# AllenNeuralDynamics/aind-smartspim-destripe

Measured on AMD Instinct MI355X. Metric: 2048x2048 uint16 slices/s destriped, higher is better.
Workload: dtype f32

## Files before the change

### aind_smartspim_destripe_amd/csrc/dsx.hip

```cpp
#include <hip/hip_runtime.h>
#include <dlfcn.h>
#include <math.h>
#include <rccl/rccl.h>
#include <stdio.h>
#include <stdlib.h>
#include <string.h>

#include <string>
#include <vector>

#include "../../include/dsx.h"
#include "dsx_kernels.h"
#include "dsx_retile.h"
#include "dsx_pyramid.h"
#include "dsx_wavelet.h"
#include "dsx_plan.h"
#include "dsx_io.h"
#include "dsx_streaks.h"
#include "dsx_zenc_kernels.h"
#include "dsx_lz4enc_kernels.h"
#include "dsx_zdec_kernels.h"

namespace {

thread_local std::string g_init_error;

enum KernelClass { KC_FWD1 = 0, KC_FWD, KC_HIST, KC_OTSU, KC_ROW, KC_INV, KC_FINAL, KC_COUNT };
const char* kClassNames[KC_COUNT] = {"k_fwd_march(level1)", "k_fwd_march(coarse)", "k_hist", "k_otsu",
                                     "k_rowfilter",       "k_inv_march(pyramid)", "k_inv_march(final)"};

struct ProfRec {
  int cls;
  hipEvent_t e0, e1;
};

}

struct DsxTuning {
  int row_wpb = 0;
  int march_waves = 256 * 16;
  bool no_quant = false;
  int seg_min_rows = 4;
  bool no_fuse = false;
  bool no_fuse_inv = false;
  bool no_pair = false;
  int hist_rows = 0;
  int fwd_wpb = 8, inv_wpb = 8;
  bool no_row_multi = false;
  int row_multi_alone = 48;
  int helper = -1;
  bool no_pipeline = false;
#ifdef DSX_DIAG
  int skip_hist = 0, skip_row = 0, skip_from = 1000;
#endif
};

struct dsx_ctx {
  int device = 0;
  DsxTuning tune;
  hipStream_t stream_ = nullptr;
  std::string err;
  bool planned = false;
  dsx::Plan plan;
  dsx::HostCfg cfg[2];
  double high_int = 2700.0;
  int max_batch = 0;
// ... 27 lines not shown
  int wl_bank_len = 0;
  bool wl_set = false;
  float wl[4][dsx::kMaxTaps] = {};
  float wl_bank[4][dsx::kMaxTaps] = {};
  unsigned* h_sticky = nullptr;
  uint8_t* zenc_slots = nullptr;
  uint32_t* zenc_sizes = nullptr;
  size_t zenc_blocks = 0;
  uint8_t* zenc_lits = nullptr;
  size_t zenc_lit_blocks = 0;
  uint8_t* zdec_scratch = nullptr;
  size_t zdec_bytes = 0;
  unsigned* d_sticky = nullptr;
  bool stack_mode = false;
  bool no_fuse_rf = false;
  bool fuse_rf_wide = false;
  int ablate = 0;
  static constexpr int kMaxStreams = 8;
  int n_streams = 4;
  hipStream_t aux[kMaxStreams] = {};
  hipEvent_t ev_fork = nullptr, ev_join[kMaxStreams] = {};
  hipStream_t helper[kMaxStreams] = {};
  hipEvent_t ev_h[kMaxStreams][4] = {};
  int joins_pending = 0;
  unsigned long long main_ops = 0;
  struct {
    const void* in = nullptr; void* out = nullptr; const void* cfg = nullptr;
    int n = 0, in_dtype = 0, out_dtype = 0, parts = 0;
    unsigned long long main_ops = 0;
  } last_split;
// ... 64 lines not shown
  t.row_wpb = env_int("DSX_ROW_WPB", 0);
  if (t.row_wpb != 0) t.row_wpb = std::max(4, std::min(t.row_wpb, (int)dsx::kRowMaxWaves));
  t.march_waves = std::max(64, env_int("DSX_MARCH_WAVES", 256 * 16));
  t.no_quant = env_int("DSX_NO_QUANT", 0) != 0;
  t.seg_min_rows = std::max(2, env_int("DSX_SEG_MIN_ROWS", 4));
  t.no_fuse = env_int("DSX_NO_FUSE", 0) != 0;
  t.no_fuse_inv = env_int("DSX_NO_FUSE_INV", 0) != 0;
  t.no_pair = env_int("DSX_NO_PAIR", 0) != 0;
  t.hist_rows = std::max(0, env_int("DSX_HIST_ROWS", 0));
  t.fwd_wpb = env_int("DSX_FWD_WPB", 8) == 4 ? 4 : 8;
  t.inv_wpb = env_int("DSX_INV_WPB", 8) == 4 ? 4 : 8;
  t.no_row_multi = env_int("DSX_NO_ROW_MULTI", 0) != 0;
  t.row_multi_alone = std::max(0, env_int("DSX_ROW_MULTI_ALONE", 48));
  t.helper = getenv("DSX_HELPER") ? (env_int("DSX_HELPER", 0) != 0 ? 1 : 0) : -1;
  t.no_pipeline = env_int("DSX_NO_PIPELINE", 0) != 0;
#ifdef DSX_DIAG
  t.skip_hist = env_int("DSX_SKIP_HIST", 0);
  t.skip_row = env_int("DSX_SKIP_ROW", 0);
  t.skip_from = env_int("DSX_SKIP_COARSE", 1000);
#endif
}

int fail(dsx_ctx* c, int code, const std::string& msg) {
  if (c) c->err = msg;
  else g_init_error = msg;
  return code;
}

hipStream_t use_main(dsx_ctx* c) {
  for (int i = 1; i < c->joins_pending; ++i) (void)hipStreamWaitEvent(c->stream_, c->ev_join[i], 0);
// ... 52 lines not shown
    }
  }
};

int rowfilter_waves_per_block(int M) {
  int best_w = 4, best_total = 0;
  for (int w = 4; w <= dsx::kRowMaxWaves; ++w) {
    const size_t bytes = (size_t)M * (w + 1) * sizeof(float2);
    const int blocks = (int)std::min<size_t>(160 * 1024 / bytes, 8);
    const int total = std::min(blocks * w, 16);
    if (total > best_total) { best_total = total; best_w = w; }
  }
  return best_w;
}

template <int CPL, int GF = -1, int NT = -1, int HALO = -1, int PLAN = 0>
hipError_t launch_rowfilter(const dsx::RowArgs& a_in, int npairs, int nb, hipStream_t s) {
  static bool attr_set[64] = {};
  int dev = 0;
  (void)hipGetDevice(&dev);
  if (!attr_set[dev & 63]) {
    hipError_t e = hipFuncSetAttribute((const void*)dsx::k_rowfilter<CPL, GF, NT, HALO, PLAN>,
                                       hipFuncAttributeMaxDynamicSharedMemorySize, 160 * 1024);
    if (e != hipSuccess) return e;
    attr_set[dev & 63] = true;
  }
  int force_wpb = tune().row_wpb;
  if (force_wpb && (size_t)a_in.M * (force_wpb + 1) * sizeof(float2) > 160 * 1024) force_wpb = 0;
  const int wpb = force_wpb ? force_wpb : ((CPL > 18 || a_in.M >= 1024) ? 4 : rowfilter_waves_per_block(a_in.M));
  const size_t smem = (size_t)a_in.M * (wpb + 1) * sizeof(float2);
  const dsx::RowArgs& a = a_in;
  const dim3 grid((npairs + wpb - 1) / wpb, nb);
  hipLaunchKernelGGL((dsx::k_rowfilter<CPL, GF, NT, HALO, PLAN>), grid, dim3(64 * wpb), smem, s, a);
  return hipGetLastError();
}

hipError_t launch_rowfilter_wide(const dsx::RowArgs& a, int npairs, int nb, hipStream_t s) {
  static bool attr_set[64] = {};
  int dev = 0;
  (void)hipGetDevice(&dev);
  if (!attr_set[dev & 63]) {
    hipError_t e = hipFuncSetAttribute((const void*)dsx::k_rowfilter_wide, hipFuncAttributeMaxDynamicSharedMemorySize,
                                       (int)(dsx::kWideMaxLen * sizeof(float2)));
    if (e != hipSuccess) return e;
    attr_set[dev & 63] = true;
  }
  if (a.M > dsx::kWideMaxLen || a.w >= 65536) return hipErrorInvalidValue;
  hipLaunchKernelGGL(dsx::k_rowfilter_wide, dim3(npairs, nb), dim3(dsx::kWideThreads), (size_t)a.M * sizeof(float2), s, a);
  return hipGetLastError();
}

hipError_t dispatch_rowfilter(const dsx::RowArgs& a, int npairs, int nb, hipStream_t s) {
  const int cpl = (a.M + 63) / 64;
  if (cpl > 36) return launch_rowfilter_wide(a, npairs, nb, s);
  const int gf = a.w >> 8, nt = (a.w - (gf << 8) + 63) >> 6;
  auto plan_is = [&](int m, int r0, int r1, int r2) {
    return a.M == m && a.npass == 3 && a.radix[0] == r0 && a.radix[1] == r1 && a.radix[2] == r2;
  };
  if (cpl <= 2) return launch_rowfilter<2>(a, npairs, nb, s);
  if (cpl <= 4) return launch_rowfilter<4>(a, npairs, nb, s);
  if (cpl <= 6) return launch_rowfilter<6>(a, npairs, nb, s);
  if (cpl <= 10) return launch_rowfilter<10>(a, npairs, nb, s);
  if (cpl <= 18) {
    if (gf == 4 && nt == 1 && a.K == 0) {
      if (plan_is(1026, 19, 9, 6))
        return launch_rowfilter<18, 4, 1, 0, 1>(a, npairs, nb, s);
      return launch_rowfilter<18, 4, 1, 0>(a, npairs, nb, s);
    }
    if (gf == 2 && nt == 1 && a.K > 0) {
      if (plan_is(1071, 17, 9, 7))
        return launch_rowfilter<18, 2, 1, 1, 2>(a, npairs, nb, s);
      return launch_rowfilter<18, 2, 1, 1>(a, npairs, nb, s);
    }
    if (gf == 1 && nt == 4 && a.K > 0) {
      if (plan_is(1024, 16, 8, 8)) return launch_rowfilter<18, 1, 4, 1, 5>(a, npairs, nb, s);
      if (plan_is(960, 15, 8, 8)) return launch_rowfilter<18, 1, 4, 1, 6>(a, npairs, nb, s);
    }
    return launch_rowfilter<18>(a, npairs, nb, s);
  }
  if (a.K > 0 && gf == 3) {
    if (nt == 4 && plan_is(2048, 16, 16, 8)) return launch_rowfilter<36, 3, 4, 1, 3>(a, npairs, nb, s);
    if (nt == 3 && plan_is(1815, 15, 11, 11)) return launch_rowfilter<36, 3, 3, 1, 4>(a, npairs, nb, s);
  }
  return launch_rowfilter<36>(a, npairs, nb, s);
}

int rowfinal_plan(const dsx::Plan& p, const dsx::LevelPlan& lp, int in_dtype, int out_dtype, bool pair_io, bool wide) {
  if (!pair_io || in_dtype != DSX_U16 || out_dtype != DSX_U16) return 0;
  if ((lp.w & 1) != 0 || (p.Wout + dsx::kMarchCols - 1) / dsx::kMarchCols > dsx::kRfWaves) return 0;
  const int gf = lp.w >> 8, nt = (lp.w - (gf << 8) + 63) >> 6;
  auto plan_is = [&](int m, int r0, int r1, int r2) {
    return lp.M == m && lp.npass == 3 && lp.radix[0] == r0 && lp.radix[1] == r1 && lp.radix[2] == r2;
  };
  if (gf == 4 && nt == 1 && lp.K == 0 && plan_is(1026, 19, 9, 6)) return 1;
  if (wide && lp.K > 0 && gf == 3 && nt == 4 && plan_is(2048, 16, 16, 8)) return 3;
  if (wide && lp.K > 0 && gf == 3 && nt == 3 && plan_is(1815, 15, 11, 11)) return 4;
  return 0;
}

template <int CPL, int GF, int NT, int HALO, int PLAN>
hipError_t launch_rowfinal_t(const dsx::RowFinalArgs& a, int nb, hipStream_t s) {
  static bool attr_set[64] = {};
  int dev = 0;
  (void)hipGetDevice(&dev);
  auto kern = dsx::k_rowfinal<CPL, GF, NT, HALO, PLAN>;
  if (!attr_set[dev & 63]) {
    hipError_t e = hipFuncSetAttribute((const void*)kern, hipFuncAttributeMaxDynamicSharedMemorySize, 160 * 1024);
    if (e != hipSuccess) return e;
    attr_set[dev & 63] = true;
  }
  const size_t smem = (size_t)a.r.M * (dsx::kRfWaves + 1) * sizeof(float2);
  const int np = (a.f.hout + 1) / 2;
  int nblk = (np + dsx::kRfRows - 1) / dsx::kRfRows;
#if DSX_RF_XCD
  nblk = (nblk + 7) / 8 * 8;
#endif
  const dim3 grid(nblk, nb);
  hipLaunchKernelGGL(kern, grid, dim3(64 * dsx::kRfWaves), smem, s, a);
  return hipGetLastError();
}

hipError_t launch_rowfinal(int plan, const dsx::RowFinalArgs& a, int nb, hipStream_t s) {
  if (plan == 1) return launch_rowfinal_t<18, 4, 1, 0, 1>(a, nb, s);
  if (plan == 3) return launch_rowfinal_t<36, 3, 4, 1, 3>(a, nb, s);
  if (plan == 4) return launch_rowfinal_t<36, 3, 3, 1, 4>(a, nb, s);
  return hipErrorInvalidValue;
}

hipError_t launch_rowfilter_multi(const dsx::RowMultiArgs& a_in, const int* npairs, int nb, hipStream_t s) {
  static bool attr_set[64] = {};
  int dev = 0;
  (void)hipGetDevice(&dev);
  if (!attr_set[dev & 63]) {
    hipError_t e = hipFuncSetAttribute((const void*)dsx::k_rowfilter_multi<6>, hipFuncAttributeMaxDynamicSharedMemorySize, 160 * 1024);
    if (e != hipSuccess) return e;
    attr_set[dev & 63] = true;
  }
  const int wpb = dsx::kRowMaxWaves;
  dsx::RowMultiArgs a = a_in;
  int blocks = 0, max_m = 1;
// ... 264 lines not shown
    a.kcut[1] = lp.kcut[1];
    a.inv_M = 1.0f / (float)lp.M;
    a.ablate = ctx->ablate;
    if (fuse_rf && l == 0) {
      row1 = a;
      continue;
    }
    const int npairs = (lp.h + 1) / 2;
    const int multi_alone = ctx->tune.row_multi_alone;
    if (!no_multi && (!v.alone || nb <= multi_alone) && rs == s && a.M <= 6 * 64 && multi.nlev < dsx::kRowMultiMax) {
      multi_pairs[multi.nlev] = npairs;
      multi.lv[multi.nlev++] = a;
      continue;
    }
    LaunchScope ls(ctx, KC_ROW);
    DSX_HIP(dispatch_rowfilter(a, npairs, nb, rs));
  }
  if (multi.nlev == 1) {
    LaunchScope ls(ctx, KC_ROW);
    DSX_HIP(dispatch_rowfilter(multi.lv[0], multi_pairs[0], nb, s));
  } else if (multi.nlev > 1) {
    LaunchScope ls(ctx, KC_ROW);
    DSX_HIP(launch_rowfilter_multi(multi, multi_pairs, nb, s));
  }
  if (split_inv) DSX_HIP(hipEventRecord(v.ev[3], v.helper));
  if (ctx->stop_after == 2) return DSX_OK;

  for (int l = L - 1; l >= (L > 0 ? 0 : -1); --l) {
    if (fuse21 && l == 1) continue;
    if (l >= skip_from) continue;
    if (generic) {
// ... 77 lines not shown
      f.has_c2 = (L > 2) ? 1 : 0;
      f.has_c = 1;
      f.pair_io = pair_io ? 1 : 0;
      if (f.rows_per_seg & 1) {
        f.rows_per_seg += 1;
        f.nseg = ((f.hout + 1) / 2 + f.rows_per_seg - 1) / f.rows_per_seg;
      }
    }
    dim3 grid((f.nstrips * f.nseg + 3) / 4, nb);
    LaunchScope ls(ctx, last ? KC_FINAL : KC_INV);
    const int inv_wpb = ctx->tune.inv_wpb;
    if (fused && fuse_rf) {
      dsx::RowFinalArgs rf;
      rf.r = row1;
      rf.f = f;
      DSX_HIP(launch_rowfinal(rf_plan, rf, nb, s));
    } else if (fused && inv_wpb == 8) {
      const dim3 g8((f.nstrips * f.nseg + 7) / 8, nb);
      if (in_dtype == DSX_U16) hipLaunchKernelGGL((dsx::k_inv_march<0, true, 8>), g8, dim3(512), 0, s, f);
      else hipLaunchKernelGGL((dsx::k_inv_march<1, true, 8>), g8, dim3(512), 0, s, f);
    } else if (fused) {
      if (in_dtype == DSX_U16) hipLaunchKernelGGL((dsx::k_inv_march<0, true>), grid, dim3(256), 0, s, f);
      else hipLaunchKernelGGL((dsx::k_inv_march<1, true>), grid, dim3(256), 0, s, f);
    } else if (!last) {
      hipLaunchKernelGGL(dsx::k_inv_march<2>, grid, dim3(256), 0, s, f);
    } else if (in_dtype == DSX_U16) {
      hipLaunchKernelGGL(dsx::k_inv_march<0>, grid, dim3(256), 0, s, f);
    } else {
      hipLaunchKernelGGL(dsx::k_inv_march<1>, grid, dim3(256), 0, s, f);
    }
    DSX_HIP(hipGetLastError());
// ... 336 lines not shown
  return DSX_OK;
}

}

extern "C" {

int dsx_device_count(void) {
  int n = 0;
  if (hipGetDeviceCount(&n) != hipSuccess) return 0;
  return n;
}

const char* dsx_last_error(const dsx_ctx* ctx) { return ctx ? ctx->err.c_str() : g_init_error.c_str(); }

int dsx_init(int device, dsx_ctx** out_ctx) {
  if (!out_ctx) { g_init_error = "out_ctx is NULL"; return DSX_EINVAL; }
  *out_ctx = nullptr;
  int n = 0;
  hipError_t e = hipGetDeviceCount(&n);
  if (e != hipSuccess || n <= 0) {
    g_init_error = std::string("no HIP device available: ") + hipGetErrorString(e);
    return DSX_EHIP;
  }
  if (device < 0 || device >= n) { g_init_error = "device index out of range"; return DSX_EINVAL; }
  e = hipSetDevice(device);
  if (e != hipSuccess) { g_init_error = std::string("hipSetDevice: ") + hipGetErrorString(e); return DSX_EHIP; }
  dsx_ctx* c = new dsx_ctx();
  c->device = device;
  read_tuning(c->tune);
// ... 117 lines not shown
  if (bank) {
    memcpy(ctx->wl, ctx->wl_bank, sizeof(ctx->wl));
    const void* fns[6] = {(const void*)dsx::k_fwd_gen<0>, (const void*)dsx::k_fwd_gen<1>, (const void*)dsx::k_fwd_gen<2>,
                          (const void*)dsx::k_inv_gen<0>, (const void*)dsx::k_inv_gen<1>, (const void*)dsx::k_inv_gen<2>};
    for (const void* fn : fns)
      DSX_HIP(hipFuncSetAttribute(fn, hipFuncAttributeMaxDynamicSharedMemorySize, 160 * 1024));
  }
  const std::string perr = dsx::build_plan(height, width, ctx->cfg, ctx->plan, bank ? ctx->wl_bank_len : dsx::kFilterLen);
  if (!perr.empty()) {
    const bool limit = perr.find("too") != std::string::npos;
    return fail(ctx, limit ? DSX_ELIMIT : DSX_EINVAL, perr);
  }
  const dsx::Plan& p = ctx->plan;
  ctx->high_int = microscope_high_int;
  ctx->max_batch = max_batch;
  const int L = p.L, Lc = L > 0 ? L : 1;

  const size_t ws_bytes = (size_t)max_batch * p.plane_floats * sizeof(float);
  DSX_HIP(hipMalloc((void**)&ctx->d_ws, ws_bytes));
  const size_t stats_b = sizeof(dsx::PlaneStats) * max_batch;
  const size_t minmax_b = sizeof(unsigned) * 2 * Lc * max_batch;
  const size_t hist_b = sizeof(unsigned) * 256 * Lc * max_batch;
  ctx->ctl_zero_bytes = stats_b + minmax_b + hist_b;
  DSX_HIP(hipMalloc((void**)&ctx->d_ctl, ctx->ctl_zero_bytes));
  ctx->d_stats = (dsx::PlaneStats*)ctx->d_ctl;
  ctx->d_minmax = (unsigned*)(ctx->d_ctl + stats_b);
  ctx->d_hist = (unsigned*)(ctx->d_ctl + stats_b + minmax_b);
  DSX_HIP(hipMalloc((void**)&ctx->d_thr, sizeof(float) * Lc * max_batch));
  DSX_HIP(hipMalloc((void**)&ctx->d_otsu, sizeof(float) * Lc * max_batch));
  DSX_HIP(hipMalloc((void**)&ctx->d_cfg, sizeof(int) * max_batch));
// ... 1116 lines not shown
```

### aind_smartspim_destripe_amd/csrc/dsx_kernels.h

```cpp
#ifndef DSX_KERNELS_H
#define DSX_KERNELS_H

#include <type_traits>
#include <hip/hip_runtime.h>
#include <stdint.h>

#include "dsx_fft_core.h"

#ifndef DSX_NT
#define DSX_NT 1
#endif
#ifndef DSX_MEDIAN_BALLOT
#define DSX_MEDIAN_BALLOT 1
#endif
#ifndef DSX_FWD_STEADY
#define DSX_FWD_STEADY 1
#endif
#ifndef DSX_RF_XCD
#define DSX_RF_XCD 0
#endif
#ifndef DSX_INV_MINW
#define DSX_INV_MINW 1
#endif
#ifndef DSX_FWD_PRUNE
// ... 1356 lines not shown
    if ((c >> 16) <= rank_b) rb = tb;
  }
  return ra | (rb << 16);
}

template <int CPL>
constexpr int row_waves_per_simd() {
  return CPL <= 18 ? 4 : 1;
}
constexpr int kRowMaxWaves = 8;

__host__ __device__ __forceinline__ constexpr int rf_lds_row_b(int M) { return (M + 1) & ~1; }

template <int CPL, int GF_, int NT_, int HALO_, int PLAN_, bool TO_LDS>
__device__ __forceinline__ void rf_pair_body(const RowArgs& a, float2* s_tw, float2* buf, int tid, int nthreads, int lane,
                                             int pair, int plane) {
  const int M = (PLAN_ > 0) ? StaticFft<PLAN_>::M : a.M;
  constexpr bool SWZ = StaticFft<PLAN_>::kSwz;
  auto P = [](int i) { return SWZ ? dsx_idx_swz::at(i) : i; };
  const int N = a.w, K = (HALO_ == 0) ? 0 : a.K;
  const bool halo = (HALO_ >= 0) ? (HALO_ != 0) : (K > 0);
  const int npairs = (a.h + 1) >> 1;
  const bool live = pair < npairs;
  const int r0 = live ? 2 * pair : 0;
  const bool has_b = (r0 + 1) < a.h;
  const int cfg = a.cfg[plane];
  float* rowa = a.ws + plane * a.ws_plane_stride + a.da_off + (long long)r0 * a.ld;
  float* rowb = rowa + a.ld;

  constexpr int GV = RowSlots<CPL>::GV;
  constexpr int E = RowSlots<CPL>::E;
// ... 27 lines not shown
    rb4[g] = make_float4(0.f, 0.f, 0.f, 0.f);
    if (active && g < gf) {
      ra4[g] = *(const float4*)(rowa + 256 * g + 4 * lane);
      if (has_b) rb4[g] = *(const float4*)(rowb + 256 * g + 4 * lane);
    }
  }
#pragma unroll
  for (int k = 0; k < 4; ++k) {
    rta[k] = 0.f;
    rtb[k] = 0.f;
    if (active && k < nt && tn + 64 * k < N) {
      rta[k] = rowa[tn + 64 * k];
      if (has_b) rtb[k] = rowb[tn + 64 * k];
    }
  }
  for (int i = tid; i < M; i += nthreads) s_tw[P(i)] = a.tw[i];
  __syncthreads();
  float* const lds_a = (float*)buf;
  float* const lds_b = (float*)buf + rf_lds_row_b(M);
  if (!active) {
    if (TO_LDS) {
      for (int n = 2 * lane; n < N; n += 2 * kWave) {
        *(float2*)(lds_a + n) = make_float2(0.f, 0.f);
        *(float2*)(lds_b + n) = make_float2(0.f, 0.f);
      }
    }
    return;
  }

  float va[E], vb[E];
  mask_t maska = 0, maskb = 0;
  auto take = [&](int e, float xa, float xb, bool valid) {
// ... 225 lines not shown
#endif
    }
  }
#pragma unroll
  for (int k = 0; k < 4; ++k) {
    const int n = tn + 64 * k;
    if (k < nt && n < N) {
      const int e = 4 * GV + k;
      const float2 y = buf[P(K + n)];
      rowa[n] = bit_select(slot_mask(maska, e), 0.f, -y.y * a.inv_M);
      if (has_b) rowb[n] = bit_select(slot_mask(maskb, e), 0.f, -y.x * a.inv_M);
    }
  }
}

template <int CPL, int GF_ = -1, int NT_ = -1, int HALO_ = -1, int PLAN_ = 0>
__global__ __launch_bounds__(64 * kRowMaxWaves, row_waves_per_simd<CPL>()) void k_rowfilter(RowArgs a) {
  extern __shared__ __attribute__((aligned(16))) float2 dsx_smem[];
  const int tid = threadIdx.x, lane = tid & 63, wave = tid >> 6;
  const int M = (PLAN_ > 0) ? StaticFft<PLAN_>::M : a.M;
  rf_pair_body<CPL, GF_, NT_, HALO_, PLAN_, false>(a, dsx_smem, dsx_smem + (long long)M * (1 + wave), tid, blockDim.x, lane,
                                                   blockIdx.x * (blockDim.x >> 6) + wave, blockIdx.y);
}

constexpr int kRowMultiMax = 8;
struct RowMultiArgs {
  int nlev;
  int blk_end[kRowMultiMax];
  RowArgs lv[kRowMultiMax];
};

template <int CPL>
__global__ __launch_bounds__(64 * kRowMaxWaves, row_waves_per_simd<CPL>()) void k_rowfilter_multi(RowMultiArgs args) {
  extern __shared__ __attribute__((aligned(16))) float2 dsx_smem[];
  const int tid = threadIdx.x, lane = tid & 63, wave = tid >> 6;
  int ent = 0;
  while (ent + 1 < args.nlev && (int)blockIdx.x >= args.blk_end[ent]) ++ent;
  const RowArgs& a = args.lv[ent];
  const int bx = (int)blockIdx.x - (ent > 0 ? args.blk_end[ent - 1] : 0);
  rf_pair_body<CPL, -1, -1, -1, 0, false>(a, dsx_smem, dsx_smem + (long long)a.M * (1 + wave), tid, blockDim.x, lane,
                                          bx * (blockDim.x >> 6) + wave, blockIdx.y);
}

constexpr int kWideThreads = 512;
constexpr int kWideCpl = 36;
constexpr int kWideMaxLen = kWideThreads * kWideCpl;

__device__ __forceinline__ unsigned wide_block_sum(unsigned v, unsigned* s_red, int& turn) {
  v = __reduce_add_sync(~0ull, v);
  unsigned* slot = s_red + ((turn & 1) ? (kWideThreads / 64) : 0);
  if ((threadIdx.x & 63) == 0) slot[threadIdx.x >> 6] = v;
  __syncthreads();
  unsigned t = 0;
#pragma unroll
  for (int w = 0; w < kWideThreads / 64; ++w) t += slot[w];
  ++turn;
// ... 669 lines not shown
  if (IN_KIND != 2 && a.flat != nullptr) {
    if (fast) inv_march_body<IN_KIND, true, IN_KIND != 2>(a, lane, strip, seg, plane);
    else inv_march_body<IN_KIND, false, IN_KIND != 2>(a, lane, strip, seg, plane);
  } else {
    if (fast) inv_march_body<IN_KIND, true, false>(a, lane, strip, seg, plane);
    else inv_march_body<IN_KIND, false, false>(a, lane, strip, seg, plane);
  }
}

constexpr int kRfWaves = 8;
constexpr int kRfRows = 2 * kRfWaves - 2;

struct RowFinalArgs {
  RowArgs r;
  FinalArgs f;
};

struct RowFinalPre {
  uint4 ni[2];

};

template <bool SHADE, bool PREFETCH_ONLY = false>
__device__ __forceinline__ void rowfinal_synth(const FinalArgs& a, const float2* smem, int M, int lane, int strip, int plane,
                                               int p_begin, int p_end, int row0, RowFinalPre& pre) {
  constexpr float RL0[6] = DSX_REC_LO;
  constexpr float RH0[6] = DSX_REC_HI;
  constexpr float KS = 1.44269504088896340736f;
  constexpr float RL[6] = {RL0[0] * KS, RL0[1] * KS, RL0[2] * KS, RL0[3] * KS, RL0[4] * KS, RL0[5] * KS};
  constexpr float RH[6] = {RH0[0] * KS, RH0[1] * KS, RH0[2] * KS, RH0[3] * KS, RH0[4] * KS, RH0[5] * KS};
// ... 152 lines not shown
    if (gyl < a.hout && x0 < a.wout)
      __builtin_amdgcn_raw_buffer_store_b128(o4, rs_out, vo_pair_out, (unsigned)(2 * p * a.wout) * 2u, kBufNT);
  };
  for (int p = p_begin; p < p_end; p += 3) {
    const bool more = p + 3 < p_end;
    step(p, ni[0], A[0], A[1], A[2], D[0], D[1], D[2]);
    if (more) ni[0] = issue_i(2 * (p + 3));
    if (p + 1 < p_end) step(p + 1, ni[1], A[1], A[2], A[0], D[1], D[2], D[0]);
    if (more) ni[1] = issue_i(2 * (p + 4));
    if (p + 2 < p_end) step(p + 2, ni[2], A[2], A[0], A[1], D[2], D[0], D[1]);
    if (more) ni[2] = issue_i(2 * (p + 5));
  }
}

template <int CPL, int GF_, int NT_, int HALO_, int PLAN_>
__global__ __launch_bounds__(64 * kRfWaves, CPL <= 18 ? 4 : 2) void k_rowfinal(RowFinalArgs a) {
  extern __shared__ __attribute__((aligned(16))) float2 dsx_smem[];
  const int tid = threadIdx.x, lane = tid & 63;
  const int wave = __builtin_amdgcn_readfirstlane(tid >> 6);
  constexpr int M = StaticFft<PLAN_>::M;
  const int plane = blockIdx.y;
#if DSX_RF_XCD
  const int per_die = gridDim.x >> 3;
  const int bx = (blockIdx.x & 7) * per_die + (blockIdx.x >> 3);
#else
  const int bx = blockIdx.x;
#endif
  const int pair0 = (kRfWaves - 1) * bx;
  rf_pair_body<CPL, GF_, NT_, HALO_, PLAN_, true>(a.r, dsx_smem, dsx_smem + (long long)M * (1 + wave), tid, 64 * kRfWaves, lane,
                                                  pair0 + wave, plane);
  const int np = (a.f.hout + 1) >> 1;
  const int p_begin = 2 * pair0, p_end = min(np, p_begin + kRfRows);
  const bool synth = wave < a.f.nstrips && p_begin < p_end;
  RowFinalPre pre;
  asm volatile("" ::: "memory");
  __builtin_amdgcn_sched_barrier(0);
  if (synth) rowfinal_synth<false, true>(a.f, dsx_smem, M, lane, wave, plane, p_begin, p_end, 2 * pair0, pre);
  __syncthreads();
  if (!synth) return;
  if (a.f.flat != nullptr) rowfinal_synth<true>(a.f, dsx_smem, M, lane, wave, plane, p_begin, p_end, 2 * pair0, pre);
  else rowfinal_synth<false>(a.f, dsx_smem, M, lane, wave, plane, p_begin, p_end, 2 * pair0, pre);
}

}
#endif
```

### aind_smartspim_destripe_amd/csrc/dsx_plan.h

```cpp
#ifndef DSX_PLAN_H
#define DSX_PLAN_H

#include <math.h>
#include <stdint.h>
#include <stdlib.h>

#include <algorithm>
#include <string>
#include <vector>

namespace dsx {

constexpr int kPlanMaxLevels = 16;
constexpr int kPlanMaxPasses = 16;
constexpr int kFilterLen = 6;
constexpr int kMaxFftLen = 64 * 36;
constexpr int kMaxWideLen = 512 * 36;

struct HostCfg {
  int level;
  double sigma;
  double max_threshold;
};

// ... 249 lines not shown
      int kc = 0;
      for (int k = 0; k < M; ++k) {
        const double mag = std::max(fabs((double)g1[k].re), sqrt((double)g2[k].re * g2[k].re + (double)g2[k].im * g2[k].im));
        if (mag > 1e-9) kc = std::max(kc, std::min(k, M - k));
      }
      lp.kcut[c] = kc;
      p.consts.insert(p.consts.end(), g1.begin(), g1.end());
      p.consts.insert(p.consts.end(), g2.begin(), g2.end());
    }
  }
  p.plane_floats = (off + 3) & ~3LL;
  if (p.plane_floats == 0) p.plane_floats = 4;
  return "";
}

}
#endif
```

### aind_smartspim_destripe_amd/engine.py

```python

import ctypes
import math
import os

import numpy as np

from . import wavelets

_HERE = os.path.dirname(os.path.abspath(__file__))
LIB_PATH = os.environ.get("DSX_LIB") or os.path.join(_HERE, "_lib", "libdsx_hip.so")

DSX_U16, DSX_F32 = 0, 1
DSX_WAVELET_DB3 = 3
DSX_WAVELET_BANK = 0
STAGE_APPROX, STAGE_DETAIL = 0, 1
STREAM_COMPUTE, STREAM_UPLOAD, STREAM_DOWNLOAD = 0, 1, 2

TASK_FILL, TASK_COPY, TASK_STORED, TASK_ZSTD, TASK_LZ4 = 0, 1, 2, 3, 4
TASK_ZLIB, TASK_BLOSCLZ = 5, 6
TASK_SHUFFLE, TASK_SPLIT, TASK_BITSHUFFLE = 0x100, 0x200, 0x400
ZDEC_ZSTD, ZDEC_ANY, ZDEC_ALL = 0, 1, 3
ROUTE_DEVICE, ROUTE_HOST, ROUTE_FILL = 0, 1, 2
TASK_DTYPE = np.dtype([("src", "<u8"), ("dst", "<u8"), ("src_len", "<u4"), ("dst_len", "<u4"), ("kind", "<u4"),
                       ("chunk", "<u4")])
# ... 7 lines not shown
    "dsx_set_shading_device", "dsx_constants_device", "dsx_run_host", "dsx_run_device", "dsx_sync",
    "dsx_malloc", "dsx_free", "dsx_memcpy_h2d", "dsx_memcpy_d2h", "dsx_memcpy_d2d",
    "dsx_timer_start", "dsx_timer_stop", "dsx_profile_enable", "dsx_profile_read",
    "dsx_get_stats", "dsx_get_thresholds", "dsx_get_level", "dsx_set_stop_after", "dsx_set_stack_mode",
    "dsx_bricks_to_planes_u16", "dsx_planes_to_bricks_u16", "dsx_downsample2_u16",
    "dsx_flatfield_correction", "dsx_flatfield_correction_rows", "dsx_foreground_background",
    "dsx_comm_unique_id", "dsx_comm_init", "dsx_comm_destroy", "dsx_comm_broadcast", "dsx_comm_allreduce_f64",
    "dsx_malloc_host", "dsx_free_host", "dsx_memcpy_h2d_async", "dsx_memcpy_d2h_async",
    "dsx_stream_wait", "dsx_stream_sync", "dsx_event_record", "dsx_event_sync",
    "dsx_io_read_chunks", "dsx_io_write_chunks", "dsx_io_write_chunks_blosc", "dsx_blosc_decode", "dsx_blosc_encode",
    "dsx_png_unfilter", "dsx_plan_streaks", "dsx_plan_streaks_ex", "dsx_get_streaks_threshold",
    "dsx_blosc_encode_device", "dsx_blosc_encode_ref", "dsx_blosc_encode_device_ex", "dsx_blosc_encode_ref_ex",
    "dsx_io_read_frames", "dsx_io_read_frames_ex", "dsx_blosc_decode_device", "dsx_blosc_decode_ref",
    "dsx_io_read_zlib_chunks", "dsx_io_write_chunks_blosc_lz4", "dsx_blosc_encode_lz4",
    "dsx_pyramid_work_bytes", "dsx_pyramid_block_u16", "dsx_pyramid_block_ref",
    "dsx_pyramid_bricks_u16", "dsx_pyramid_bricks_ref",
]


def frame_tasks_per_chunk(chunk_bytes):
    return int(chunk_bytes) // 8192 + 1


def decode_task(src, dst, src_len, dst_len, kind, chunk=0):
    t = np.zeros(1, TASK_DTYPE)
    t[0] = (src, dst, src_len, dst_len, kind, chunk)
    return t


class DsxError(RuntimeError):

# ... 134 lines not shown
    lib.dsx_blosc_encode_ref_ex.argtypes = [vp, i32, ctypes.c_size_t, i32, i32, vp, vp, i32]
    lib.dsx_io_read_frames.argtypes = [vp, ctypes.POINTER(ctypes.c_char_p), i32, ctypes.c_size_t, i32, ctypes.c_uint16,
                                       vp, ctypes.c_size_t, vp, i32, ctypes.POINTER(ctypes.c_size_t),
                                       ctypes.POINTER(i32), vp]
    lib.dsx_io_read_frames_ex.argtypes = lib.dsx_io_read_frames.argtypes + [i32]
    lib.dsx_io_read_zlib_chunks.argtypes = lib.dsx_io_read_frames.argtypes
    lib.dsx_blosc_decode_device.argtypes = [vp, vp, ctypes.c_size_t, vp, i32, vp, ctypes.c_size_t, vp]
    lib.dsx_blosc_decode_ref.argtypes = [vp, ctypes.c_size_t, vp, i32, vp, ctypes.c_size_t, vp]
    lib.dsx_pyramid_work_bytes.argtypes = [i32, i32, i32, i32, ctypes.POINTER(ctypes.c_size_t)]
    lib.dsx_pyramid_block_u16.argtypes = [vp, vp, i32, i32, i32, i32, ctypes.POINTER(_PyramidLevel), ctypes.POINTER(vp),
                                          vp, ctypes.c_size_t]
    lib.dsx_pyramid_block_ref.argtypes = [vp, i32, i32, i32, i32, ctypes.POINTER(_PyramidLevel), ctypes.POINTER(vp)]
    lib.dsx_pyramid_bricks_u16.argtypes = [vp, vp] + [i32] * 7 + [ctypes.POINTER(_PyramidLevel), ctypes.POINTER(vp), vp,
                                                                  ctypes.c_size_t]
    lib.dsx_pyramid_bricks_ref.argtypes = [vp] + [i32] * 7 + [ctypes.POINTER(_PyramidLevel), ctypes.POINTER(vp)]
    for name in EXPORTED_SYMBOLS:
        fn = getattr(lib, name)
        if name not in ("dsx_destroy", "dsx_last_error"):
            fn.restype = ctypes.c_int
    if path is None:
        _lib = lib
    return lib


STREAKS_ROUTES = {"generic": 0, "march": 1}
AUTO_ROUTE = "generic"


def _db3_max_level(height, width):
    def one(n):
# ... 654 lines not shown
```

### include/dsx.h

```cpp
#ifndef DSX_H
#define DSX_H

#include <stddef.h>
#include <stdint.h>

#ifdef __cplusplus
extern "C" {
#endif

#define DSX_VERSION 100

#define DSX_OK 0
#define DSX_EINVAL (-1)
#define DSX_ENOPLAN (-2)
#define DSX_EHIP (-3)
#define DSX_ENOMEM (-4)
#define DSX_ELIMIT (-5)
#define DSX_ECOMM (-6)
#define DSX_EIO (-7)
#define DSX_EVALUE (-8)

#define DSX_U16 0
#define DSX_F32 1

// ... 32 lines not shown
             const dsx_cfg* no_cells_config, double microscope_high_int, const float* flat,
             const float* dark, int dark_h, int dark_w);
int dsx_plan_info(const dsx_ctx* ctx, dsx_plan_info_t* info);
int dsx_set_wavelet(dsx_ctx* ctx, const double* dec_lo, const double* dec_hi, const double* rec_lo,
                    const double* rec_hi, int len);
int dsx_set_shading_device(dsx_ctx* ctx, const float* d_flat, const float* d_dark, int dark_h,
                           int dark_w);
int dsx_constants_device(const dsx_ctx* ctx, void** d_ptr, size_t* bytes);

int dsx_run_host(dsx_ctx* ctx, const void* in, int in_dtype, int n, void* out, int out_dtype,
                 int32_t* cfg_used);
int dsx_run_device(dsx_ctx* ctx, const void* d_in, int in_dtype, int n, void* d_out,
                   int out_dtype, int32_t* d_cfg_used);
int dsx_sync(dsx_ctx* ctx);
int dsx_graph_stats(const dsx_ctx* ctx, uint64_t* launches, uint64_t* captures);

int dsx_malloc(dsx_ctx* ctx, size_t bytes, void** d_ptr);
int dsx_free(dsx_ctx* ctx, void* d_ptr);
int dsx_memcpy_h2d(dsx_ctx* ctx, void* d_dst, const void* src, size_t bytes);
int dsx_memcpy_d2h(dsx_ctx* ctx, void* dst, const void* d_src, size_t bytes);
int dsx_memcpy_d2d(dsx_ctx* ctx, void* d_dst, const void* d_src, size_t bytes);
#define DSX_STREAM_COMPUTE 0
#define DSX_STREAM_UPLOAD 1
#define DSX_STREAM_DOWNLOAD 2
int dsx_malloc_host(dsx_ctx* ctx, size_t bytes, void** h_ptr);
int dsx_free_host(dsx_ctx* ctx, void* h_ptr);
int dsx_memcpy_h2d_async(dsx_ctx* ctx, void* d_dst, const void* src, size_t bytes, int stream_id);
int dsx_memcpy_d2h_async(dsx_ctx* ctx, void* dst, const void* d_src, size_t bytes, int stream_id);
int dsx_stream_wait(dsx_ctx* ctx, int waiter, int signaller);
int dsx_stream_sync(dsx_ctx* ctx, int stream_id);
// ... 124 lines not shown
```

Baseline: 69640.

## Add grid-stride tile loop to row filter kernels with occupancy-capped grid option

Converts the planned row-filter and fused row-final kernels from a 2D (tile, plane) grid to a 1D tile index loop, so a block can process several tiles. The grid can be capped at the device's resident-block capacity, which is queried once at plan time. Twiddle loading into LDS is skipped after a block's first tile, to amortize setup and launch cost. The default setting keeps one tile per block, so the persistent mode is opt-in. It adds per-tile index math and an extra barrier between iterations.

```diff
diff --git a/aind_smartspim_destripe_amd/csrc/dsx.hip b/aind_smartspim_destripe_amd/csrc/dsx.hip
--- a/aind_smartspim_destripe_amd/csrc/dsx.hip
+++ b/aind_smartspim_destripe_amd/csrc/dsx.hip
@@ -36,6 +36,9 @@
 
 }
 
+#ifndef DSX_RF_TILES_DEFAULT
+#define DSX_RF_TILES_DEFAULT 1
+#endif
 struct DsxTuning {
   int row_wpb = 0;
   int march_waves = 256 * 16;
@@ -50,6 +53,7 @@
   int row_multi_alone = 48;
   int helper = -1;
   bool no_pipeline = false;
+  int rf_tiles = DSX_RF_TILES_DEFAULT;
 #ifdef DSX_DIAG
   int skip_hist = 0, skip_row = 0, skip_from = 1000;
 #endif
@@ -107,6 +111,7 @@
   unsigned* d_sticky = nullptr;
   bool stack_mode = false;
   bool no_fuse_rf = false;
+  int rf_cap_final = 0, rf_cap_row[2] = {0, 0};
   bool fuse_rf_wide = false;
   int ablate = 0;
   static constexpr int kMaxStreams = 8;
@@ -201,6 +206,7 @@
   t.row_multi_alone = std::max(0, env_int("DSX_ROW_MULTI_ALONE", 48));
   t.helper = getenv("DSX_HELPER") ? (env_int("DSX_HELPER", 0) != 0 ? 1 : 0) : -1;
   t.no_pipeline = env_int("DSX_NO_PIPELINE", 0) != 0;
+  t.rf_tiles = std::max(0, std::min(env_int("DSX_RF_TILES", DSX_RF_TILES_DEFAULT), 1 << 20));
 #ifdef DSX_DIAG
   t.skip_hist = env_int("DSX_SKIP_HIST", 0);
   t.skip_row = env_int("DSX_SKIP_ROW", 0);
@@ -283,8 +289,16 @@
   return best_w;
 }
 
+int resident_blocks(const void* kern, int threads, size_t smem) {
+  int dev = 0, per_cu = 0;
+  hipDeviceProp_t prop;
+  if (hipGetDevice(&dev) != hipSuccess || hipGetDeviceProperties(&prop, dev) != hipSuccess) return 0;
+  if (hipOccupancyMaxActiveBlocksPerMultiprocessor(&per_cu, kern, threads, smem) != hipSuccess) return 0;
+  return std::max(0, per_cu) * std::max(0, prop.multiProcessorCount);
+}
+
 template <int CPL, int GF = -1, int NT = -1, int HALO = -1, int PLAN = 0>
-hipError_t launch_rowfilter(const dsx::RowArgs& a_in, int npairs, int nb, hipStream_t s) {
+hipError_t launch_rowfilter(const dsx::RowArgs& a_in, int npairs, int nb, hipStream_t s, int cap, int* cap_query) {
   static bool attr_set[64] = {};
   int dev = 0;
   (void)hipGetDevice(&dev);
@@ -299,8 +313,16 @@
   const int wpb = force_wpb ? force_wpb : ((CPL > 18 || a_in.M >= 1024) ? 4 : rowfilter_waves_per_block(a_in.M));
   const size_t smem = (size_t)a_in.M * (wpb + 1) * sizeof(float2);
   const dsx::RowArgs& a = a_in;
-  const dim3 grid((npairs + wpb - 1) / wpb, nb);
-  hipLaunchKernelGGL((dsx::k_rowfilter<CPL, GF, NT, HALO, PLAN>), grid, dim3(64 * wpb), smem, s, a);
+  if (cap_query) {
+    *cap_query = PLAN > 0 ? resident_blocks((const void*)dsx::k_rowfilter<CPL, GF, NT, HALO, PLAN>, 64 * wpb, smem) : 0;
+    return hipSuccess;
+  }
+  dsx::RowTileArgs ta;
+  ta.r = a;
+  ta.tl.per_plane = (npairs + wpb - 1) / wpb;
+  ta.tl.total = ta.tl.per_plane * nb;
+  const dim3 grid = PLAN > 0 ? dim3(dsx::rf_grid(ta.tl.total, tune().rf_tiles, cap)) : dim3(ta.tl.per_plane, nb);
+  hipLaunchKernelGGL((dsx::k_rowfilter<CPL, GF, NT, HALO, PLAN>), grid, dim3(64 * wpb), smem, s, ta);
   return hipGetLastError();
 }
 
@@ -319,39 +341,42 @@
   return hipGetLastError();
 }
 
-hipError_t dispatch_rowfilter(const dsx::RowArgs& a, int npairs, int nb, hipStream_t s) {
+hipError_t dispatch_rowfilter(const dsx::RowArgs& a, int npairs, int nb, hipStream_t s, int cap = 0, int* cap_query = nullptr) {
   const int cpl = (a.M + 63) / 64;
-  if (cpl > 36) return launch_rowfilter_wide(a, npairs, nb, s);
+  if (cpl > 36) {
+    if (cap_query) return *cap_query = 0, hipSuccess;
+    return launch_rowfilter_wide(a, npairs, nb, s);
+  }
   const int gf = a.w >> 8, nt = (a.w - (gf << 8) + 63) >> 6;
   auto plan_is = [&](int m, int r0, int r1, int r2) {
     return a.M == m && a.npass == 3 && a.radix[0] == r0 && a.radix[1] == r1 && a.radix[2] == r2;
   };
-  if (cpl <= 2) return launch_rowfilter<2>(a, npairs, nb, s);
-  if (cpl <= 4) return launch_rowfilter<4>(a, npairs, nb, s);
-  if (cpl <= 6) return launch_rowfilter<6>(a, npairs, nb, s);
-  if (cpl <= 10) return launch_rowfilter<10>(a, npairs, nb, s);
+  if (cpl <= 2) return launch_rowfilter<2>(a, npairs, nb, s, cap, cap_query);
+  if (cpl <= 4) return launch_rowfilter<4>(a, npairs, nb, s, cap, cap_query);
+  if (cpl <= 6) return launch_rowfilter<6>(a, npairs, nb, s, cap, cap_query);
+  if (cpl <= 10) return launch_rowfilter<10>(a, npairs, nb, s, cap, cap_query);
   if (cpl <= 18) {
     if (gf == 4 && nt == 1 && a.K == 0) {
       if (plan_is(1026, 19, 9, 6))
-        return launch_rowfilter<18, 4, 1, 0, 1>(a, npairs, nb, s);
-      return launch_rowfilter<18, 4, 1, 0>(a, npairs, nb, s);
+        return launch_rowfilter<18, 4, 1, 0, 1>(a, npairs, nb, s, cap, cap_query);
+      return launch_rowfilter<18, 4, 1, 0>(a, npairs, nb, s, cap, cap_query);
     }
     if (gf == 2 && nt == 1 && a.K > 0) {
       if (plan_is(1071, 17, 9, 7))
-        return launch_rowfilter<18, 2, 1, 1, 2>(a, npairs, nb, s);
-      return launch_rowfilter<18, 2, 1, 1>(a, npairs, nb, s);
+        return launch_rowfilter<18, 2, 1, 1, 2>(a, npairs, nb, s, cap, cap_query);
+      return launch_rowfilter<18, 2, 1, 1>(a, npairs, nb, s, cap, cap_query);
     }
     if (gf == 1 && nt == 4 && a.K > 0) {
-      if (plan_is(1024, 16, 8, 8)) return launch_rowfilter<18, 1, 4, 1, 5>(a, npairs, nb, s);
-      if (plan_is(960, 15, 8, 8)) return launch_rowfilter<18, 1, 4, 1, 6>(a, npairs, nb, s);
-    }
-    return launch_rowfilter<18>(a, npairs, nb, s);
+      if (plan_is(1024, 16, 8, 8)) return launch_rowfilter<18, 1, 4, 1, 5>(a, npairs, nb, s, cap, cap_query);
+      if (plan_is(960, 15, 8, 8)) return launch_rowfilter<18, 1, 4, 1, 6>(a, npairs, nb, s, cap, cap_query);
+    }
+    return launch_rowfilter<18>(a, npairs, nb, s, cap, cap_query);
   }
   if (a.K > 0 && gf == 3) {
-    if (nt == 4 && plan_is(2048, 16, 16, 8)) return launch_rowfilter<36, 3, 4, 1, 3>(a, npairs, nb, s);
-    if (nt == 3 && plan_is(1815, 15, 11, 11)) return launch_rowfilter<36, 3, 3, 1, 4>(a, npairs, nb, s);
-  }
-  return launch_rowfilter<36>(a, npairs, nb, s);
+    if (nt == 4 && plan_is(2048, 16, 16, 8)) return launch_rowfilter<36, 3, 4, 1, 3>(a, npairs, nb, s, cap, cap_query);
+    if (nt == 3 && plan_is(1815, 15, 11, 11)) return launch_rowfilter<36, 3, 3, 1, 4>(a, npairs, nb, s, cap, cap_query);
+  }
+  return launch_rowfilter<36>(a, npairs, nb, s, cap, cap_query);
 }
 
 int rowfinal_plan(const dsx::Plan& p, const dsx::LevelPlan& lp, int in_dtype, int out_dtype, bool pair_io, bool wide) {
@@ -368,7 +393,8 @@
 }
 
 template <int CPL, int GF, int NT, int HALO, int PLAN>
-hipError_t launch_rowfinal_t(const dsx::RowFinalArgs& a, int nb, hipStream_t s) {
+hipError_t launch_rowfinal_t(const dsx::RowFinalArgs& a_in, int nb, hipStream_t s, int cap, int* cap_query) {
+  dsx::RowFinalArgs a = a_in;
   static bool attr_set[64] = {};
   int dev = 0;
   (void)hipGetDevice(&dev);
@@ -379,20 +405,29 @@
     attr_set[dev & 63] = true;
   }
   const size_t smem = (size_t)a.r.M * (dsx::kRfWaves + 1) * sizeof(float2);
+  if (cap_query) {
+    *cap_query = resident_blocks((const void*)kern, 64 * dsx::kRfWaves, smem);
+    return hipSuccess;
+  }
   const int np = (a.f.hout + 1) / 2;
   int nblk = (np + dsx::kRfRows - 1) / dsx::kRfRows;
 #if DSX_RF_XCD
   nblk = (nblk + 7) / 8 * 8;
 #endif
-  const dim3 grid(nblk, nb);
-  hipLaunchKernelGGL(kern, grid, dim3(64 * dsx::kRfWaves), smem, s, a);
+  a.tl.per_plane = nblk;
+  a.tl.total = nblk * nb;
+  int blocks = dsx::rf_grid(a.tl.total, tune().rf_tiles, cap);
+#if DSX_RF_XCD
+  blocks = std::min(a.tl.total, (blocks + 7) / 8 * 8);
+#endif
+  hipLaunchKernelGGL(kern, dim3(blocks), dim3(64 * dsx::kRfWaves), smem, s, a);
   return hipGetLastError();
 }
 
-hipError_t launch_rowfinal(int plan, const dsx::RowFinalArgs& a, int nb, hipStream_t s) {
-  if (plan == 1) return launch_rowfinal_t<18, 4, 1, 0, 1>(a, nb, s);
-  if (plan == 3) return launch_rowfinal_t<36, 3, 4, 1, 3>(a, nb, s);
-  if (plan == 4) return launch_rowfinal_t<36, 3, 3, 1, 4>(a, nb, s);
+hipError_t launch_rowfinal(int plan, const dsx::RowFinalArgs& a, int nb, hipStream_t s, int cap, int* cap_query = nullptr) {
+  if (plan == 1) return launch_rowfinal_t<18, 4, 1, 0, 1>(a, nb, s, cap, cap_query);
+  if (plan == 3) return launch_rowfinal_t<36, 3, 4, 1, 3>(a, nb, s, cap, cap_query);
+  if (plan == 4) return launch_rowfinal_t<36, 3, 3, 1, 4>(a, nb, s, cap, cap_query);
   return hipErrorInvalidValue;
 }
 
@@ -687,7 +722,7 @@
       continue;
     }
     LaunchScope ls(ctx, KC_ROW);
-    DSX_HIP(dispatch_rowfilter(a, npairs, nb, rs));
+    DSX_HIP(dispatch_rowfilter(a, npairs, nb, rs, l < 2 ? ctx->rf_cap_row[l] : 0));
   }
   if (multi.nlev == 1) {
     LaunchScope ls(ctx, KC_ROW);
@@ -795,7 +830,7 @@
       dsx::RowFinalArgs rf;
       rf.r = row1;
       rf.f = f;
-      DSX_HIP(launch_rowfinal(rf_plan, rf, nb, s));
+      DSX_HIP(launch_rowfinal(rf_plan, rf, nb, s, ctx->rf_cap_final));
     } else if (fused && inv_wpb == 8) {
       const dim3 g8((f.nstrips * f.nseg + 7) / 8, nb);
       if (in_dtype == DSX_U16) hipLaunchKernelGGL((dsx::k_inv_march<0, true, 8>), g8, dim3(512), 0, s, f);
@@ -1162,6 +1197,8 @@
 
 const char* dsx_last_error(const dsx_ctx* ctx) { return ctx ? ctx->err.c_str() : g_init_error.c_str(); }
 
+int dsx_rf_grid(int tiles, int rf_tiles, int capacity) { return dsx::rf_grid(tiles, std::max(0, rf_tiles), capacity); }
+
 int dsx_init(int device, dsx_ctx** out_ctx) {
   if (!out_ctx) { g_init_error = "out_ctx is NULL"; return DSX_EINVAL; }
   *out_ctx = nullptr;
@@ -1309,6 +1346,26 @@
   const dsx::Plan& p = ctx->plan;
   ctx->high_int = microscope_high_int;
   ctx->max_batch = max_batch;
+  {
+    ctx->rf_cap_final = ctx->rf_cap_row[0] = ctx->rf_cap_row[1] = 0;
+    for (int l = 0; l < 2 && l < p.L; ++l) {
+      const dsx::LevelPlan& lp = p.lv[l];
+      dsx::RowArgs a;
+      memset(&a, 0, sizeof(a));
+      a.w = lp.w; a.M = lp.M; a.K = lp.K;
+      a.npass = lp.npass;
+      for (int i = 0; i < lp.npass; ++i) a.radix[i] = lp.radix[i];
+      t_tune = &ctx->tune;
+      DSX_HIP(dispatch_rowfilter(a, 0, 0, nullptr, 0, &ctx->rf_cap_row[l]));
+    }
+    const int rf_plan = p.L >= 2 ? rowfinal_plan(p, p.lv[0], DSX_U16, DSX_U16, true, ctx->fuse_rf_wide) : 0;
+    if (rf_plan != 0) {
+      dsx::RowFinalArgs rf;
+      memset(&rf, 0, sizeof(rf));
+      rf.r.M = p.lv[0].M;
+      DSX_HIP(launch_rowfinal(rf_plan, rf, 0, nullptr, 0, &ctx->rf_cap_final));
+    }
+  }
   const int L = p.L, Lc = L > 0 ? L : 1;
 
   const size_t ws_bytes = (size_t)max_batch * p.plane_floats * sizeof(float);
diff --git a/aind_smartspim_destripe_amd/csrc/dsx_kernels.h b/aind_smartspim_destripe_amd/csrc/dsx_kernels.h
--- a/aind_smartspim_destripe_amd/csrc/dsx_kernels.h
+++ b/aind_smartspim_destripe_amd/csrc/dsx_kernels.h
@@ -1394,7 +1394,7 @@
 
 template <int CPL, int GF_, int NT_, int HALO_, int PLAN_, bool TO_LDS>
 __device__ __forceinline__ void rf_pair_body(const RowArgs& a, float2* s_tw, float2* buf, int tid, int nthreads, int lane,
-                                             int pair, int plane) {
+                                             int pair, int plane, bool& tw_ready) {
   const int M = (PLAN_ > 0) ? StaticFft<PLAN_>::M : a.M;
   constexpr bool SWZ = StaticFft<PLAN_>::kSwz;
   auto P = [](int i) { return SWZ ? dsx_idx_swz::at(i) : i; };
@@ -1452,8 +1452,11 @@
       if (has_b) rtb[k] = rowb[tn + 64 * k];
     }
   }
-  for (int i = tid; i < M; i += nthreads) s_tw[P(i)] = a.tw[i];
-  __syncthreads();
+  if (!tw_ready) {
+    for (int i = tid; i < M; i += nthreads) s_tw[P(i)] = a.tw[i];
+    __syncthreads();
+    tw_ready = true;
+  }
   float* const lds_a = (float*)buf;
   float* const lds_b = (float*)buf + rf_lds_row_b(M);
   if (!active) {
@@ -1709,13 +1712,51 @@
   }
 }
 
+struct RowTiles {
+  int per_plane, total;
+};
+__device__ __forceinline__ void row_tile(int t, const RowTiles& tl, int& plane, int& bx) {
+  asm volatile("" : "+s"(t));
+  plane = __builtin_amdgcn_readfirstlane((int)((unsigned)t / (unsigned)tl.per_plane));
+  bx = t - plane * tl.per_plane;
+}
+template <class ARGS>
+__device__ __forceinline__ const ARGS& row_tile_args() {
+  auto p = __builtin_amdgcn_kernarg_segment_ptr();
+  asm volatile("" : "+s"(p));
+  return *(const ARGS*)p;
+}
+__device__ __forceinline__ int row_tile_lane() {
+  unsigned all = ~0u;
+  asm volatile("" : "+s"(all));
+  return (int)__builtin_amdgcn_mbcnt_hi(all, __builtin_amdgcn_mbcnt_lo(all, 0u));
+}
+struct RowTileArgs {
+  RowArgs r;
+  RowTiles tl;
+};
+
 template <int CPL, int GF_ = -1, int NT_ = -1, int HALO_ = -1, int PLAN_ = 0>
-__global__ __launch_bounds__(64 * kRowMaxWaves, row_waves_per_simd<CPL>()) void k_rowfilter(RowArgs a) {
+__global__ __launch_bounds__(64 * kRowMaxWaves, row_waves_per_simd<CPL>()) void k_rowfilter(RowTileArgs args) {
   extern __shared__ __attribute__((aligned(16))) float2 dsx_smem[];
-  const int tid = threadIdx.x, lane = tid & 63, wave = tid >> 6;
+  const RowArgs& a = args.r;
   const int M = (PLAN_ > 0) ? StaticFft<PLAN_>::M : a.M;
-  rf_pair_body<CPL, GF_, NT_, HALO_, PLAN_, false>(a, dsx_smem, dsx_smem + (long long)M * (1 + wave), tid, blockDim.x, lane,
-                                                   blockIdx.x * (blockDim.x >> 6) + wave, blockIdx.y);
+  bool tw_ready = false;
+  if constexpr (PLAN_ > 0) {
+    const int wave = __builtin_amdgcn_readfirstlane(threadIdx.x >> 6);
+    for (int t = blockIdx.x; t < args.tl.total; t += gridDim.x) {
+      const RowTileArgs& ta = row_tile_args<RowTileArgs>();
+      const int lane = row_tile_lane(), tid = 64 * wave + lane;
+      int plane, bx;
+      row_tile(t, ta.tl, plane, bx);
+      rf_pair_body<CPL, GF_, NT_, HALO_, PLAN_, false>(ta.r, dsx_smem, dsx_smem + (long long)M * (1 + wave), tid, blockDim.x,
+                                                       lane, bx * (blockDim.x >> 6) + wave, plane, tw_ready);
+    }
+  } else {
+    const int tid = threadIdx.x, lane = tid & 63, wave = tid >> 6;
+    rf_pair_body<CPL, GF_, NT_, HALO_, PLAN_, false>(a, dsx_smem, dsx_smem + (long long)M * (1 + wave), tid, blockDim.x, lane,
+                                                     blockIdx.x * (blockDim.x >> 6) + wave, blockIdx.y, tw_ready);
+  }
 }
 
 constexpr int kRowMultiMax = 8;
@@ -1733,8 +1774,9 @@
   while (ent + 1 < args.nlev && (int)blockIdx.x >= args.blk_end[ent]) ++ent;
   const RowArgs& a = args.lv[ent];
   const int bx = (int)blockIdx.x - (ent > 0 ? args.blk_end[ent - 1] : 0);
+  bool tw_ready = false;
   rf_pair_body<CPL, -1, -1, -1, 0, false>(a, dsx_smem, dsx_smem + (long long)a.M * (1 + wave), tid, blockDim.x, lane,
-                                          bx * (blockDim.x >> 6) + wave, blockIdx.y);
+                                          bx * (blockDim.x >> 6) + wave, blockIdx.y, tw_ready);
 }
 
 constexpr int kWideThreads = 512;
@@ -2434,6 +2476,7 @@
 struct RowFinalArgs {
   RowArgs r;
   FinalArgs f;
+  RowTiles tl;
 };
 
 struct RowFinalPre {
@@ -2616,32 +2659,44 @@
 }
 
 template <int CPL, int GF_, int NT_, int HALO_, int PLAN_>
-__global__ __launch_bounds__(64 * kRfWaves, CPL <= 18 ? 4 : 2) void k_rowfinal(RowFinalArgs a) {
+__global__ __launch_bounds__(64 * kRfWaves, CPL <= 18 ? 4 : 2) void k_rowfinal(RowFinalArgs args) {
   extern __shared__ __attribute__((aligned(16))) float2 dsx_smem[];
-  const int tid = threadIdx.x, lane = tid & 63;
-  const int wave = __builtin_amdgcn_readfirstlane(tid >> 6);
   constexpr int M = StaticFft<PLAN_>::M;
-  const int plane = blockIdx.y;
+  bool tw_ready = false;
+  const int wave = __builtin_amdgcn_readfirstlane(threadIdx.x >> 6);
+  for (int t = blockIdx.x; t < args.tl.total; t += gridDim.x) {
+    const RowFinalArgs& a = row_tile_args<RowFinalArgs>();
+    const int lane = row_tile_lane(), tid = 64 * wave + lane;
+    int plane, bx;
+    row_tile(t, a.tl, plane, bx);
 #if DSX_RF_XCD
-  const int per_die = gridDim.x >> 3;
-  const int bx = (blockIdx.x & 7) * per_die + (blockIdx.x >> 3);
-#else
-  const int bx = blockIdx.x;
+    bx = (bx & 7) * (a.tl.per_plane >> 3) + (bx >> 3);
 #endif
-  const int pair0 = (kRfWaves - 1) * bx;
-  rf_pair_body<CPL, GF_, NT_, HALO_, PLAN_, true>(a.r, dsx_smem, dsx_smem + (long long)M * (1 + wave), tid, 64 * kRfWaves, lane,
-                                                  pair0 + wave, plane);
-  const int np = (a.f.hout + 1) >> 1;
-  const int p_begin = 2 * pair0, p_end = min(np, p_begin + kRfRows);
-  const bool synth = wave < a.f.nstrips && p_begin < p_end;
-  RowFinalPre pre;
-  asm volatile("" ::: "memory");
-  __builtin_amdgcn_sched_barrier(0);
-  if (synth) rowfinal_synth<false, true>(a.f, dsx_smem, M, lane, wave, plane, p_begin, p_end, 2 * pair0, pre);
-  __syncthreads();
-  if (!synth) return;
-  if (a.f.flat != nullptr) rowfinal_synth<true>(a.f, dsx_smem, M, lane, wave, plane, p_begin, p_end, 2 * pair0, pre);
-  else rowfinal_synth<false>(a.f, dsx_smem, M, lane, wave, plane, p_begin, p_end, 2 * pair0, pre);
+    const int pair0 = (kRfWaves - 1) * bx;
+    rf_pair_body<CPL, GF_, NT_, HALO_, PLAN_, true>(a.r, dsx_smem, dsx_smem + (long long)M * (1 + wave), tid, 64 * kRfWaves,
+                                                    lane, pair0 + wave, plane, tw_ready);
+    const int np = (a.f.hout + 1) >> 1;
+    const int p_begin = 2 * pair0, p_end = min(np, p_begin + kRfRows);
+    const bool synth = wave < a.f.nstrips && p_begin < p_end;
+    RowFinalPre pre;
+    pre.ni[0] = pre.ni[1] = make_uint4(0u, 0u, 0u, 0u);
+    asm volatile("" ::: "memory");
+    __builtin_amdgcn_sched_barrier(0);
+    if (synth) rowfinal_synth<false, true>(a.f, dsx_smem, M, lane, wave, plane, p_begin, p_end, 2 * pair0, pre);
+    __syncthreads();
+    if (synth) {
+      int ls = lane;
+      if (a.f.flat != nullptr) {
+        asm volatile("" : "+v"(ls));
+        rowfinal_synth<true>(a.f, dsx_smem, M, ls, wave, plane, p_begin, p_end, 2 * pair0, pre);
+      } else {
+        asm volatile("" : "+v"(ls));
+        rowfinal_synth<false>(a.f, dsx_smem, M, ls, wave, plane, p_begin, p_end, 2 * pair0, pre);
+      }
+    }
+    if (t + (int)gridDim.x >= a.tl.total) break;
+    __syncthreads();
+  }
 }
 
 }
diff --git a/aind_smartspim_destripe_amd/csrc/dsx_plan.h b/aind_smartspim_destripe_amd/csrc/dsx_plan.h
--- a/aind_smartspim_destripe_amd/csrc/dsx_plan.h
+++ b/aind_smartspim_destripe_amd/csrc/dsx_plan.h
@@ -287,5 +287,11 @@
   return "";
 }
 
+inline int rf_grid(int tiles, int rf_tiles, int capacity) {
+  tiles = std::max(tiles, 1);
+  if (rf_tiles <= 0) return capacity > 0 ? std::min(tiles, capacity) : tiles;
+  return (int)(((long long)tiles + rf_tiles - 1) / rf_tiles);
+}
+
 }
 #endif
diff --git a/aind_smartspim_destripe_amd/engine.py b/aind_smartspim_destripe_amd/engine.py
--- a/aind_smartspim_destripe_amd/engine.py
+++ b/aind_smartspim_destripe_amd/engine.py
@@ -45,7 +45,7 @@
     "dsx_io_read_frames", "dsx_io_read_frames_ex", "dsx_blosc_decode_device", "dsx_blosc_decode_ref",
     "dsx_io_read_zlib_chunks", "dsx_io_write_chunks_blosc_lz4", "dsx_blosc_encode_lz4",
     "dsx_pyramid_work_bytes", "dsx_pyramid_block_u16", "dsx_pyramid_block_ref",
-    "dsx_pyramid_bricks_u16", "dsx_pyramid_bricks_ref",
+    "dsx_pyramid_bricks_u16", "dsx_pyramid_bricks_ref", "dsx_rf_grid",
 ]
 
 
@@ -210,6 +210,7 @@
     lib.dsx_pyramid_bricks_u16.argtypes = [vp, vp] + [i32] * 7 + [ctypes.POINTER(_PyramidLevel), ctypes.POINTER(vp), vp,
                                                                   ctypes.c_size_t]
     lib.dsx_pyramid_bricks_ref.argtypes = [vp] + [i32] * 7 + [ctypes.POINTER(_PyramidLevel), ctypes.POINTER(vp)]
+    lib.dsx_rf_grid.argtypes = [i32, i32, i32]
     for name in EXPORTED_SYMBOLS:
         fn = getattr(lib, name)
         if name not in ("dsx_destroy", "dsx_last_error"):
diff --git a/include/dsx.h b/include/dsx.h
--- a/include/dsx.h
+++ b/include/dsx.h
@@ -70,6 +70,7 @@
                    int out_dtype, int32_t* d_cfg_used);
 int dsx_sync(dsx_ctx* ctx);
 int dsx_graph_stats(const dsx_ctx* ctx, uint64_t* launches, uint64_t* captures);
+int dsx_rf_grid(int tiles, int rf_tiles, int capacity);
 
 int dsx_malloc(dsx_ctx* ctx, size_t bytes, void** d_ptr);
 int dsx_free(dsx_ctx* ctx, void* d_ptr);
```

Result: slower. 67870 (-2.5%).
